# RunhuiWang/DeltaPQ

Measured on AMD Instinct MI355X. Metric: queries/sec, SIFT1M-shaped m=8 k=256 topk=100, higher is better.
Workload: dtype f64 sum of f32 table entries (u8 code decode; the reference's incremental f64 stack); 1 GPU

## Files before the change

deltapq_amd/csrc/dpq_kernels.hip:

```cpp
#include "dpq_kernels.h"
#include "dpq_wave_decoder.h"

#include <atomic>
#include <type_traits>
#include <cfloat>
#include <cmath>

namespace dpq {

static hipError_t ensure_dynamic_lds(const void* fn, size_t bytes, std::atomic<bool>* done);


__device__ __forceinline__ uint32_t and_or(uint32_t a, uint32_t mask, uint32_t c) {
    uint32_t r;
    asm("v_and_or_b32 %0, %1, %2, %3" : "=v"(r) : "v"(a), "s"(mask), "v"(c));
    return r;
}

__device__ __forceinline__ uint64_t make_key(float d, uint32_t id) {
    return ((uint64_t)__float_as_uint(d) << 32) | (uint64_t)id;
}

__device__ __forceinline__ float lut_min_of(const float* __restrict__ lut_min, size_t q, int M, int m) {
    const float4 p = *reinterpret_cast<const float4*>(lut_min + (q * M + m) * kLutMinParts);
// ... 66 lines not shown
    }
}

template <int M>
__global__ __launch_bounds__(64) void decode_segments_kernel(const DeviceImage img,
                                                              const uint32_t* __restrict__ seg_list,
                                                              uint32_t* __restrict__ out_id,
                                                              uint32_t* __restrict__ out_code) {
    constexpr int W = Cfg<M>::W;
    const int lane = threadIdx.x;
    const uint32_t seg = seg_list ? seg_list[blockIdx.x] : blockIdx.x;
    const int cps = img.chunks_per_segment;
    WaveDecoder<M> dec;
    if (!img.raw) dec.begin_segment(img, seg, lane);
    for (int c = 0; c < cps; ++c) {
        const int64_t node = ((int64_t)seg * cps + c) * 64 + lane;
        uint32_t code[W];
        if (img.raw) {
#pragma unroll
            for (int w = 0; w < W; ++w) code[w] = reinterpret_cast<const uint32_t*>(img.raw)[(size_t)node * W + w];
        } else {
            dec.step(img, node, lane, c + 1 < cps, code);
        }
        const size_t o = ((size_t)blockIdx.x * cps + c) * 64 + lane;
        out_id[o] = node < img.n_local ? img.id_base + (uint32_t)node : 0xffffffffu;
#pragma unroll
        for (int w = 0; w < W; ++w) out_code[W * o + w] = code[w];
    }
}

template <int M>
__global__ __launch_bounds__(256) void decode_list_kernel(const DeviceImage img, const uint32_t* __restrict__ seg_list,
                                                           int n_seg, const uint8_t* __restrict__ relabel,
                                                           uint32_t* __restrict__ out_code) {
    constexpr int W = Cfg<M>::W;
    __builtin_amdgcn_s_setprio(DPQ_UNDER_SCAN_PRIO);
    const int lane = threadIdx.x & 63;
    const int64_t j = (int64_t)blockIdx.x * 4 + (threadIdx.x >> 6);
    if (j >= n_seg) return;
    const int64_t seg = seg_list ? (int64_t)seg_list[j] : j;
    const int cps = img.chunks_per_segment;
    WaveDecoder<M> dec;
    dec.begin_segment(img, (uint32_t)seg, lane);
    for (int c = 0; c < cps; ++c) {
        const int64_t node = (seg * cps + c) * 64 + lane;
        const int64_t out = (j * cps + c) * 64 + lane;
        uint32_t code[W];
        dec.step(img, node, lane, c + 1 < cps, code);
        if (relabel) {
#pragma unroll
            for (int w = 0; w < W; ++w) {
                uint32_t r = 0;
#pragma unroll
                for (int b = 0; b < 4; ++b) r |= (uint32_t)relabel[(4 * w + b) * 256 + ((code[w] >> (8 * b)) & 0xffu)] << (8 * b);
                code[w] = r;
            }
        }
        if constexpr (W == 2)
            reinterpret_cast<uint2*>(out_code)[out] = make_uint2(code[0], code[1]);
        else
            reinterpret_cast<uint4*>(out_code)[out] = make_uint4(code[0], code[1], code[2], code[3]);
    }
}

template <int M>
__device__ __forceinline__ float exact_dist(const float* __restrict__ T, const uint32_t* __restrict__ c, bool fp32_accum) {
    if (fp32_accum) {
        float fsum = 0.0f;
#pragma unroll
        for (int m = 0; m < M; ++m) fsum = __fadd_rn(fsum, T[m * 256 + ((c[m >> 2] >> (8 * (m & 3))) & 0xffu)]);
        return fsum;
    }
    double dsum = 0.0;
#pragma unroll
    for (int m = 0; m < M; ++m) {
        const uint32_t byte = (c[m >> 2] >> (8 * (m & 3))) & 0xffu;
        dsum = __dadd_rn(dsum, (double)T[m * 256 + byte]);
    }
    return (float)dsum;
}

struct FilterScale {
    float s32;
    uint32_t bias;
    double B;
};

template <int M>
__device__ __forceinline__ FilterScale filter_scale(uint64_t key, const float* __restrict__ lut_min, size_t q) {
    using C = Cfg<M>;
    FilterScale r{0.0f, 0u, 0.0};
    double B = 0.0;
#pragma unroll
    for (int mm = 0; mm < M; ++mm) B += (double)lut_min_of(lut_min, q, M, mm);
    const double taup = (double)__uint_as_float((uint32_t)(key >> 32)) * (1.0 + 0x1p-20);
    const double R = taup - B;
    r.B = B;
    if (key != ~0ull && R > 0.0 && R < 1e300) {
        const float s = (float)((double)C::QT / R * (1.0 - 0x1p-20));
        if (s <= FLT_MAX) {
            r.s32 = s;
            r.bias = C::R == 1 ? (uint32_t)C::BIAS : 0u;
        }
    }
    return r;
}

template <int M>
__device__ __forceinline__ float filter_offset(const FilterScale& fs, float min_m, int m) {
    const float mn = fs.s32 != 0.0f ? min_m : 0.0f;
    const double od = (double)mn * (double)fs.s32;
    float of = (float)od;
    if ((double)of < od) of = __uint_as_float(__float_as_uint(of) + 1u);
    const double sd = (m == 0 ? (double)fs.bias : 0.0) - 0.5 - (double)of;
    float sf = (float)sd;
    if ((double)sf > sd) sf = __uint_as_float(__float_as_uint(sf) + (sf > 0.0f ? -1 : 1));
    return sf;
}

template <int M>
__device__ __forceinline__ uint32_t filter_field(float tv, float sc, float of, uint32_t bias_m) {
    using C = Cfg<M>;
    const float fv = fminf(__fmaf_rn(tv, sc, of), (float)C::SAT + (float)bias_m);
    return __builtin_amdgcn_cvt_pk_u8_f32(fv, 0u, 0u);
}

template <int M>
__device__ __forceinline__ void write_filter_fields(uint4* qtab, int slot, const float* T, float sc, const float* of_m,
                                                    uint32_t bias, const uint8_t* __restrict__ relabel, int tid, int nthreads) {
    using C = Cfg<M>;
    constexpr int F = C::F, AB = C::AB, R = C::R, QG = C::QG, NG = C::NG, J = C::J;
    const int group = slot / QG, ls = slot % QG;
    const int f = (ls % (J * F)) / J, acc = (ls / (J * F)) * AB + ls % J;
    const int d = acc / R, tb = f * R + acc % R;
    const int g = d >> 2, c = d & 3;
    unsigned char* base = reinterpret_cast<unsigned char*>(qtab + ((size_t)group * NG + g) * M * 256) + c * 4 + tb;
    for (int e = tid; e < M * 256; e += nthreads) {
        const int m = e >> 8;
        const uint32_t v = T ? filter_field<M>(T[e], sc, of_m[m], m == 0 ? bias : 0u) : C::reject_entry(m);
        const int row = relabel ? (m << 8) + relabel[e] : e;
        base[(size_t)row * 16] = (unsigned char)v;
    }
}

template <int M>
__global__ __launch_bounds__(256) void quantise_kernel(const ScanArgs a) {
    using C = Cfg<M>;
    constexpr int QG = C::QG, NG = C::NG;
    constexpr int TE = M * 256;
    constexpr int NS = 16;
    __shared__ float s_scale[NS], s_off[NS];
    __shared__ int32_t s_row[NS];
    __shared__ uint32_t s_bias[NS];
    const int g = blockIdx.x / M, m = blockIdx.x % M, group = blockIdx.y, k = threadIdx.x;
    if (blockIdx.x == 0 && a.tight_hist)
        for (int i = k; i < QG * kTightWords; i += 256) a.tight_hist[(size_t)group * QG * kTightWords + i] = 0;
    if (k < NS) {
        const int ls = C::slot_of_table(g, k >> 2, k & 3);
        const int slot = group * QG + ls;
        int qq = a.slot_query ? a.slot_query[slot] : (slot < a.n_queries ? slot : -1);
        FilterScale fs{0.0f, 0u, 0.0};
        float mn_m = 0.0f;
        if (qq >= 0 && a.debug_pass != 1) {
            uint64_t key = ~0ull;
            if (a.debug_pass != 2) key = a.thr_key[slot];
            fs = filter_scale<M>(key, a.lut_min, (size_t)qq);
            mn_m = lut_min_of(a.lut_min, (size_t)qq, M, m);
        } else {
            qq = -1;
        }
        const float s32 = fs.s32;
        const uint32_t bias = fs.bias;
        const float of = filter_offset<M>(fs, mn_m, m);
        s_scale[k] = s32;
        s_off[k] = of;
        s_bias[k] = m == 0 ? bias : 0u;
        s_row[k] = qq >= 0 ? qq * TE + m * 256 : -1;
    }
    __syncthreads();
    uint32_t out[4] = {0, 0, 0, 0};
#pragma unroll
    for (int c = 0; c < 4; ++c) {
#pragma unroll
        for (int tb = 0; tb < 4; ++tb) {
            const int i = c * 4 + tb;
            const int row = s_row[i];
            const float sc = s_scale[i], of = s_off[i];
            const uint32_t bias = s_bias[i];
            const float tv = row >= 0 ? a.lut32[(size_t)row + k] : 0.0f;
            const float fv = fminf(__fmaf_rn(tv, sc, of), (float)C::SAT + (float)bias);
            out[c] = row < 0 ? out[c] | (C::reject_entry(m) << (8 * tb))
                             : __builtin_amdgcn_cvt_pk_u8_f32(fv, (uint32_t)tb, out[c]);
        }
    }
    a.qtab[((size_t)group * NG * M + blockIdx.x) * 256 + k] = make_uint4(out[0], out[1], out[2], out[3]);
}

#ifndef DPQ_TIGHT_SLEEP
#define DPQ_TIGHT_SLEEP 32
#endif
#ifndef DPQ_GATHER_PIPE
#define DPQ_GATHER_PIPE 0
#endif

constexpr int kFiltered = 0x1000;

template <int M>
struct ScanLds {
    using C = Cfg<M>;
    static constexpr size_t kTables = (size_t)C::NG * M * 256 * 16;
    static constexpr size_t kThr = kTables;
    static constexpr size_t kBase = kThr + (size_t)C::QG * 8;
    static constexpr size_t kCount = kBase + (size_t)C::QG * 4;
    static constexpr size_t kChecks = kCount + (size_t)C::QG * 4;
    static constexpr size_t kScale = kChecks + 16;
    static constexpr size_t kBdn = kScale + (size_t)C::QG * 4;
    static constexpr size_t kExtra = kBdn + (size_t)C::QG * 4;
    static constexpr size_t kHist = kExtra + (size_t)C::NA * 4;
    static constexpr size_t kQCode = kHist + (size_t)C::QG * kTightBuckets * 2;
    static constexpr size_t kQId = kQCode + (size_t)kScanWaves * C::QCAP * M;
    static constexpr size_t kQMask = kQId + (size_t)kScanWaves * C::QCAP * 4;
    static constexpr size_t kBytes = kQMask + (size_t)kScanWaves * C::QCAP * 4 * C::MD;
    static_assert(kBytes <= 160 * 1024, "one workgroup per CU: 160 KB of LDS");
};

enum { kStPrologue = 0, kStSegment, kStDecode, kStGather, kStFold, kStPush, kStRefine, kStTotal, kStSteps, kStRefines,
       kStWaves, kStEntries, kStCount };

template <int MF, bool PLAIN, bool STAMPS, bool TIGHT>
__global__ __launch_bounds__(kScanThreads, (PLAIN && !STAMPS && (MF & ~kFiltered) <= 8) ? 5 : 4) void scan_kernel(const ScanArgs a) {
    constexpr int M = MF & ~kFiltered;
    constexpr bool FILT = (MF & kFiltered) != 0;
    using C = Cfg<M>;
    constexpr int W = C::W, QG = C::QG, NG = C::NG, NA = C::NA, EB = C::AB, F = C::F, MD = C::MD, QCAP = C::QCAP;
    constexpr int TE = M * 256;
    extern __shared__ __attribute__((aligned(16))) unsigned char smem[];
    uint4* lut = reinterpret_cast<uint4*>(smem);
    uint64_t* s_thr = reinterpret_cast<uint64_t*>(smem + ScanLds<M>::kThr);
    int32_t* s_base = reinterpret_cast<int32_t*>(smem + ScanLds<M>::kBase);
    uint32_t* wg_count = reinterpret_cast<uint32_t*>(smem + ScanLds<M>::kCount);
    uint32_t* wg_checks = reinterpret_cast<uint32_t*>(smem + ScanLds<M>::kChecks);
    uint32_t* wg_next = wg_checks + 1;
    float* s_scale = reinterpret_cast<float*>(smem + ScanLds<M>::kScale);
    float* s_bdn = reinterpret_cast<float*>(smem + ScanLds<M>::kBdn);
    uint32_t* s_extra = reinterpret_cast<uint32_t*>(smem + ScanLds<M>::kExtra);
    uint32_t* s_hist = reinterpret_cast<uint32_t*>(smem + ScanLds<M>::kHist);
    uint32_t* rq_code = reinterpret_cast<uint32_t*>(smem + ScanLds<M>::kQCode) + (size_t)(threadIdx.x >> 6) * QCAP * W;
    uint32_t* rq_id = reinterpret_cast<uint32_t*>(smem + ScanLds<M>::kQId) + (size_t)(threadIdx.x >> 6) * QCAP;
    uint32_t* rq_mask = reinterpret_cast<uint32_t*>(smem + ScanLds<M>::kQMask) + (size_t)(threadIdx.x >> 6) * QCAP * MD;

    const int tid = threadIdx.x;
    const int lane = tid & 63;
    uint64_t st[kStCount] = {};
    uint64_t t_mark = 0, t_start = 0;
    auto stamp = [&](int section) {
        if constexpr (STAMPS) {
            const uint64_t now = __builtin_amdgcn_s_memtime();
            st[section] += now - t_mark;
            t_mark = now;
// ... 254 lines not shown
            if (k.c == 0) {
                k.h_doff = a.img.seg_delta_off[k.seg];
#pragma unroll
                for (int w = 0; w < W; ++w) k.h_stk[w] = 0;
                if (lane < C::LEVELS) {
                    const uint32_t* ck = reinterpret_cast<const uint32_t*>(a.img.seg_ckpt) + ((size_t)k.seg * C::LEVELS + lane) * W;
#pragma unroll
                    for (int w = 0; w < W; ++w) k.h_stk[w] = ck[w];
                }
            }
        }
    };
    uint64_t at = 0;
    auto stage2 = [&](Chunk& k) {
        if (k.seg < 0 || PLAIN) return;
        if (k.c == 0) at = k.h_doff;
        k.ld = WaveDecoder<M>::load_delta(a.img, k.in, node_of(k), at);
    };
    auto successor = [&](const Chunk& k) {
        Chunk n;
        n.seg = k.seg;
        n.pos = k.pos;
        n.c = k.c + 1;
        if (k.seg >= 0 && n.c == cps) {
            n.seg = next_entry();
            n.pos = entry_pos;
            n.c = 0;
        }
        return n;
    };
    Chunk A, B, Cn;
    uint32_t fwA = 0, fwB = 0, fwC = 0;
    auto filter_word = [&](const Chunk& k) -> uint32_t { return k.seg < 0 ? 0u : a.filter[(size_t)node_of(k) >> 5]; };
    A.seg = helper ? -1 : next_entry();
    A.pos = entry_pos;
    A.c = 0;
    stage1(A);
    if constexpr (FILT) fwA = filter_word(A);
    B = successor(A);
    stage1(B);
    if constexpr (FILT) fwB = filter_word(B);
    stage2(A);
    stamp(kStSegment);
    while (A.seg >= 0) {
        if constexpr (PLAIN) {
#pragma unroll
            for (int w = 0; w < W; ++w) asm volatile("" ::"v"(A.raw[w]), "v"(B.raw[w]));
        } else {
            asm volatile("" ::"v"(A.ld.level), "v"(A.ld.mk), "v"(A.ld.par), "v"(A.carry_lane), "v"(B.in.nb), "v"(B.in.mk),
                         "v"(B.in.par), "v"(B.carry_lane));
#pragma unroll
            for (int h = 0; h < W / 2; ++h)
                asm volatile("" ::"v"(A.ld.w[h][0]), "v"(A.ld.w[h][1]), "v"(A.ld.w[h][2]), "v"(A.ld.t[h].x), "v"(A.ld.t[h].y));
#pragma unroll
            for (int w = 0; w < W; ++w) asm volatile("" ::"v"(A.h_stk[w]), "v"(B.h_stk[w]));
        }
        if constexpr (FILT) asm volatile("" ::"v"(fwA), "v"(fwB));
        Cn = successor(B);
        stage2(B);
        stage1(Cn);
        if constexpr (FILT) fwC = filter_word(Cn);
        {
            const int64_t node = node_of(A);
            uint32_t code[W];
            if (PLAIN) {
#pragma unroll
                for (int w = 0; w < W; ++w) code[w] = A.raw[w];
            } else {
                if (A.c == 0) {
#pragma unroll
                    for (int w = 0; w < W; ++w) dec.stk[w] = A.h_stk[w];
                }
                dec.finish(A.ld, lane, A.carry_lane, code);
            }
            if constexpr (STAMPS) {
                st[kStSteps] += 1;
                asm volatile("" ::"v"(code[0]), "v"(code[W - 1]));
            }
            stamp(kStDecode);

            uint32_t acc[NA];
            uint32_t fold_h[MD] = {};
            if constexpr (C::R == 1 && DPQ_GATHER_PIPE > 0) {
                static_assert(NG * 8 == 32 && (DPQ_GATHER_PIPE % 2) == 0 && DPQ_GATHER_PIPE >= 2 && DPQ_GATHER_PIPE <= 14, "window of read pairs");
                uint32_t off[8];
#pragma unroll
                for (int m = 0; m < 8; ++m) off[m] = (code[m >> 2] >> (8 * (m & 3))) & 0xffu;
                uint4 gv[32];
#define DPQ_RD(r) gv[r] = lut[(((r) >> 3) * M + ((r) & 7)) * 256 + off[(r) & 7]]
#pragma unroll
                for (int r = 0; r < DPQ_GATHER_PIPE; r += 2) {
                    DPQ_RD(r);
                    DPQ_RD(r + 1);
                    __builtin_amdgcn_sched_barrier(0);
                }
#pragma unroll
                for (int p = 0; p < 16; ++p) {
                    if (2 * p + DPQ_GATHER_PIPE < 32) {
                        DPQ_RD(2 * p + DPQ_GATHER_PIPE);
                        DPQ_RD(2 * p + DPQ_GATHER_PIPE + 1);
                    }
                    __builtin_amdgcn_sched_barrier(0);
                    const int g = p >> 2;
                    const uint4 x = gv[2 * p], y = gv[2 * p + 1];
                    if ((p & 3) == 0) {
                        acc[4 * g + 0] = x.x + y.x;
                        acc[4 * g + 1] = x.y + y.y;
                        acc[4 * g + 2] = x.z + y.z;
                        acc[4 * g + 3] = x.w + y.w;
                    } else {
                        acc[4 * g + 0] += x.x + y.x;
                        acc[4 * g + 1] += x.y + y.y;
                        acc[4 * g + 2] += x.z + y.z;
                        acc[4 * g + 3] += x.w + y.w;
                    }
                    if ((p & 3) == 3) {
#pragma unroll
                        for (int j = 4 * g; j < 4 * g + 4; ++j)
                            fold_h[j / EB] = and_or(acc[j], C::LOW << (EB - 1), fold_h[j / EB] >> 1);
                    }
                    __builtin_amdgcn_sched_barrier(0);
                }
#undef DPQ_RD
            } else
#pragma unroll
            for (int g = 0; g < NG; ++g) {
                if constexpr (C::R == 1) {
                    uint4 v[8];
#pragma unroll
                    for (int m = 0; m < 8; ++m) {
                        const uint32_t byte = (code[m >> 2] >> (8 * (m & 3))) & 0xffu;
                        v[m] = lut[(g * M + m) * 256 + byte];
                    }
                    acc[4 * g + 0] = ((v[0].x + v[1].x + v[2].x) + v[3].x + v[4].x) + (v[5].x + v[6].x + v[7].x);
                    acc[4 * g + 1] = ((v[0].y + v[1].y + v[2].y) + v[3].y + v[4].y) + (v[5].y + v[6].y + v[7].y);
                    acc[4 * g + 2] = ((v[0].z + v[1].z + v[2].z) + v[3].z + v[4].z) + (v[5].z + v[6].z + v[7].z);
                    acc[4 * g + 3] = ((v[0].w + v[1].w + v[2].w) + v[3].w + v[4].w) + (v[5].w + v[6].w + v[7].w);
                } else {
                    uint32_t lo[4], hi[4];
                    if constexpr (TIGHT) {
                        asm volatile("" ::: "memory");
                        const uint4 e0 = reinterpret_cast<const uint4*>(s_extra)[2 * g], e1 = reinterpret_cast<const uint4*>(s_extra)[2 * g + 1];
                        lo[0] = e0.x, hi[0] = e0.y, lo[1] = e0.z, hi[1] = e0.w, lo[2] = e1.x, hi[2] = e1.y, lo[3] = e1.z, hi[3] = e1.w;
                    } else {
#pragma unroll
                        for (int c = 0; c < 4; ++c) lo[c] = hi[c] = (uint32_t)C::BIAS * C::LOW;
                    }
#pragma unroll
                    for (int m0 = 0; m0 < M; m0 += C::PRE) {
                        uint32_t p[4] = {0, 0, 0, 0};
#pragma unroll
                        for (int mm = 0; mm < C::PRE; ++mm) {
                            const int m = m0 + mm;
                            const uint32_t byte = (code[m >> 2] >> (8 * (m & 3))) & 0xffu;
                            const uint4 v = lut[(g * M + m) * 256 + byte];
                            p[0] += v.x, p[1] += v.y, p[2] += v.z, p[3] += v.w;
                        }
#pragma unroll
                        for (int c = 0; c < 4; ++c) {
                            lo[c] += __builtin_amdgcn_perm(0u, p[c], 0x0c020c00u);
                            hi[c] += __builtin_amdgcn_perm(0u, p[c], 0x0c030c01u);
                        }
                    }
#pragma unroll
                    for (int c = 0; c < 4; ++c) {
                        acc[(4 * g + c) * 2 + 0] = lo[c];
                        acc[(4 * g + c) * 2 + 1] = hi[c];
                    }
                }
            }
            if constexpr (STAMPS) {
#pragma unroll
                for (int i = 0; i < NA; ++i) asm volatile("" ::"v"(acc[i]));
            }
            stamp(kStGather);
            bool valid = node < a.img.n_local;
            if constexpr (FILT) valid = valid && ((fwA >> ((uint32_t)node & 31u)) & 1u) != 0u;
            uint64_t pend = 0;
#pragma unroll
            for (int h = 0; h < MD; ++h) {
                uint32_t fail = 0;
                if constexpr (C::R == 1 && DPQ_GATHER_PIPE > 0) {
                    fail = fold_h[h];
                } else {
#pragma unroll
                    for (int j = 0; j < C::J; ++j) fail = and_or(acc[EB * h + j], C::LOW << (EB - 1), fail >> 1);
                }
                fail >>= EB - C::J;
                pend |= (uint64_t)(valid ? (~fail & live) : 0u) << (32 * h);
            }
            const uint64_t pushing = __ballot(pend != 0);
            stamp(kStFold);
            if (pushing) {
                const int cnt = (int)__popcll(pushing);
                while (rq_n + cnt > QCAP) {
                    refine(min(rq_n, 64));
                    stamp(kStRefine);
                }
                if (pend != 0) {
                    int pos = rq_head + rq_n + (int)mbcnt64(pushing, 0);
                    pos = pos >= QCAP ? pos - QCAP : pos;
#pragma unroll
                    for (int w = 0; w < W; ++w) rq_code[pos * W + w] = code[w];
                    rq_id[pos] = a.img.id_base + (uint32_t)node;
                    rq_mask[pos * MD] = (uint32_t)pend;
                    if constexpr (MD == 2) rq_mask[pos * MD + 1] = (uint32_t)(pend >> 32);
                }
                rq_n += cnt;
                stamp(kStPush);
            }
        }
        A = B;
        B = Cn;
        if constexpr (FILT) fwA = fwB, fwB = fwC;
    }
    while (rq_n > 0) refine(min(rq_n, 64));
    stamp(kStRefine);
    if constexpr (TIGHT) {
        if (helper) {
            for (;;) {
// ... 377 lines not shown
#define DPQ_S1_SKIP 0
#endif
#ifndef DPQ_S1_U8
#define DPQ_S1_U8 1
#endif
#ifndef DPQ_S1_PAIR
#define DPQ_S1_PAIR 2
#endif
#ifndef DPQ_S1_DEPTH
#define DPQ_S1_DEPTH 1
#endif
#ifndef DPQ_S1_THREADS
#define DPQ_S1_THREADS 1024
#endif
constexpr int kS1Threads = DPQ_S1_THREADS, kS1Waves = kS1Threads / 64;
constexpr int kS1Buckets = 64;
static_assert((DPQ_S1_QT >> 2) < kS1Buckets && DPQ_S1_QT <= 253, "a lane per bucket; 8 entries of 255 must reject");

struct S1Lds {
    static constexpr size_t kTq = 0;
    static constexpr size_t kSel = kTq + 256 * 32 * 8;
    static constexpr size_t kStack = kSel + 16 * 32 * 4;
    static constexpr size_t kT32 = kStack + (size_t)kS1Waves * 8 * 64 * 8;
    static constexpr size_t kShare = kT32 + 8 * 256 * 4;
    static constexpr size_t kHist = kShare + 48;
    static constexpr size_t kBytes = kHist + 64 * 4;
};
static_assert(S1Lds::kBytes <= 160 * 1024 && S1Lds::kTq == 0, "one workgroup per CU; the bound rows sit at LDS offset 0");

#define DPQ_LDS __attribute__((address_space(3)))
__device__ __forceinline__ uint2 lds_ld64(uint32_t off) {
    const uint64_t v = *(const DPQ_LDS uint64_t*)(uintptr_t)off;
    return make_uint2((uint32_t)v, (uint32_t)(v >> 32));
}
__device__ __forceinline__ uint32_t lds_ld32(uint32_t off) { return *(const DPQ_LDS uint32_t*)(uintptr_t)off; }
__device__ __forceinline__ void lds_st64(uint32_t off, uint2 v) { *(DPQ_LDS uint64_t*)(uintptr_t)off = ((uint64_t)v.y << 32) | v.x; }
__device__ __forceinline__ uint32_t lds_ld8(uint32_t off) { return *(const DPQ_LDS uint8_t*)(uintptr_t)off; }
__device__ __forceinline__ uint2 lds_ld64_whole(uint32_t off) {
    const uint64_t v = *(const volatile DPQ_LDS uint64_t*)(uintptr_t)off;
    return make_uint2((uint32_t)v, (uint32_t)(v >> 32));
}

__device__ __forceinline__ uint32_t s1_nibble_sel(uint32_t nib) {
    uint32_t sel = 0, rank = 0;
#pragma unroll
    for (int i = 0; i < 4; ++i) {
        const bool set = (nib >> i) & 1u;
        sel |= (set ? rank : 4u + i) << (8 * i);
        rank += set ? 1u : 0u;
    }
    return sel;
}

__device__ __forceinline__ uint32_t wave_inclusive_sum(uint32_t v) {
    v += (uint32_t)__builtin_amdgcn_update_dpp(0, (int)v, 0x111, 0xf, 0xf, false);
    v += (uint32_t)__builtin_amdgcn_update_dpp(0, (int)v, 0x112, 0xf, 0xf, false);
    v += (uint32_t)__builtin_amdgcn_update_dpp(0, (int)v, 0x114, 0xf, 0xf, false);
    v += (uint32_t)__builtin_amdgcn_update_dpp(0, (int)v, 0x118, 0xf, 0xf, false);
    v += (uint32_t)__builtin_amdgcn_update_dpp(0, (int)v, 0x142, 0xa, 0xf, false);
    v += (uint32_t)__builtin_amdgcn_update_dpp(0, (int)v, 0x143, 0xc, 0xf, false);
    return v;
}

__global__ __launch_bounds__(kS1Threads) void strand1_kernel(const ScanArgs a) {
    constexpr int M = 8, TE = M * 256, GROUPS = kRunLen / kPhaseLen, D = DPQ_S1_DEPTH, QT = DPQ_S1_QT;
    extern __shared__ __attribute__((aligned(16))) unsigned char smem[];
    const int tid = threadIdx.x, lane = tid & 63, wave = tid >> 6;
    const int slot = blockIdx.y;
    const int qq = a.slot_query ? (slot < a.n_queries ? a.slot_query[slot] : -1) : (slot < a.n_queries ? slot : -1);
    if (qq < 0) return;
    if ((uint32_t)(uintptr_t)(DPQ_LDS unsigned char*)smem != 0u) __builtin_trap();
    uint64_t thr = a.thr_key[slot];
    unsigned long long* const stp = a.stamps ? a.stamps + ((size_t)blockIdx.x * kS1Waves + wave) * 16 : nullptr;
    int n_stamp = 0;
    unsigned long long slow_ticks = 0, slow_entries = 0;
    auto stamp = [&]() {
        if (stp && n_stamp < 14) {
            const unsigned long long t = (__builtin_amdgcn_s_memrealtime() & 0xffffffffffull) | ((__builtin_amdgcn_s_memtime() >> 10) << 40);
            if (lane == 0) stp[n_stamp] = t;
            ++n_stamp;
        }
    };
    stamp();
    FilterScale fs{0.0f, 0u, 0.0};
    float min_m[M];
    {
        double B = 0.0;
#pragma unroll
        for (int m = 0; m < M; ++m) {
            min_m[m] = lut_min_of(a.lut_min, (size_t)qq, M, m);
            B += (double)min_m[m];
        }
        const double taup = (double)__uint_as_float((uint32_t)(thr >> 32)) * (1.0 + 0x1p-20);
        const double R = taup - B;
        fs.B = B;
        if (thr != ~0ull && R > 0.0 && R < 1e300) fs.s32 = (float)((double)QT / R * (1.0 - 0x1p-20));
        if (!(fs.s32 <= FLT_MAX)) fs.s32 = 0.0f;
    }
    const float sc = fs.s32, bdn = __double2float_rd(fs.B);
    const int dbg = a.debug_pass >= 16 ? a.debug_pass - 16 : 0;
    uint32_t* hist = a.tight_hist && sc != 0.0f && !(dbg & 4) ? a.tight_hist + (size_t)slot * (kS1Replicas * kS1ReplicaWords) : nullptr;
    int cut = QT;

    float* T32 = reinterpret_cast<float*>(smem + S1Lds::kT32);
    {
        const float* src = a.lut32 + (size_t)qq * TE;
        for (int i = tid; i < TE; i += kS1Threads) T32[i] = src[i];
        if (tid < 16 * 32) reinterpret_cast<uint32_t*>(smem + S1Lds::kSel)[tid] = s1_nibble_sel((uint32_t)tid >> 5);
        __syncthreads();
        uint2* qtmp = reinterpret_cast<uint2*>(smem + S1Lds::kStack);
        if (tid < 256) {
            uint32_t lo = 0, hi = 0;
#pragma unroll
            for (int m = 0; m < M; ++m) {
                const float of = filter_offset<M>(fs, min_m[m], 1);
                const float fv = sc != 0.0f ? fminf(__fmaf_rn(T32[m * 256 + tid], sc, of), 255.0f) : 0.0f;
                if (m < 4)
                    lo = __builtin_amdgcn_cvt_pk_u8_f32(fv, (uint32_t)m, lo);
                else
                    hi = __builtin_amdgcn_cvt_pk_u8_f32(fv, (uint32_t)(m - 4), hi);
            }
            qtmp[tid] = make_uint2(lo, hi);
        }
        __syncthreads();
        uint2* Tq = reinterpret_cast<uint2*>(smem + S1Lds::kTq);
        if constexpr (DPQ_S1_U8) {
            uint32_t* Tw = reinterpret_cast<uint32_t*>(smem + S1Lds::kTq);
            for (int w = tid; w < 256 * 64; w += kS1Threads) {
                const uint2 row = qtmp[w >> 6];
                Tw[w] = ((w >> 5) & 1) ? row.y : row.x;
            }
        } else {
            for (int w = tid; w < 256 * 32; w += kS1Threads) Tq[w] = qtmp[w >> 5];
        }
        if (tid == 0) {
            *reinterpret_cast<uint32_t*>(smem + S1Lds::kShare) = (uint32_t)QT;
            *reinterpret_cast<unsigned long long*>(smem + S1Lds::kShare + 8) = thr;
            *reinterpret_cast<uint4*>(smem + S1Lds::kShare + 16) = make_uint4(0u, 0u, 0u, 0u);
            *reinterpret_cast<uint4*>(smem + S1Lds::kShare + 32) = make_uint4(0u, 0u, 0u, 0u);
        }
        if (tid < 64) reinterpret_cast<uint32_t*>(smem + S1Lds::kHist)[tid] = 0u;
        __syncthreads();
    }

    stamp();
    const uint32_t lane8 = (uint32_t)(lane & 31) * (DPQ_S1_U8 ? 4u : 8u);
    const uint32_t lane_sel = (uint32_t)S1Lds::kSel + (uint32_t)(lane & 31) * 4u;
    const uint32_t lane_stk = (uint32_t)S1Lds::kStack + (uint32_t)wave * (8 * 64 * 8) + (uint32_t)lane * 8u - 512u;

    DPQ_LDS uint32_t* const sh_cut = (DPQ_LDS uint32_t*)(uintptr_t)S1Lds::kShare;
    DPQ_LDS unsigned long long* const sh_thr = (DPQ_LDS unsigned long long*)(uintptr_t)(S1Lds::kShare + 8);
    DPQ_LDS uint32_t* const sh_count = (DPQ_LDS uint32_t*)(uintptr_t)(S1Lds::kShare + 16);
    DPQ_LDS uint32_t* const sh_done = (DPQ_LDS uint32_t*)(uintptr_t)(S1Lds::kShare + 20);
    DPQ_LDS uint32_t* const sh_next = (DPQ_LDS uint32_t*)(uintptr_t)(S1Lds::kShare + 24);
    DPQ_LDS uint32_t* const sh_stat = (DPQ_LDS uint32_t*)(uintptr_t)(S1Lds::kShare + 32);
    DPQ_LDS uint32_t* const sh_hist = (DPQ_LDS uint32_t*)(uintptr_t)S1Lds::kHist;
    auto look = [&]() {
        const uint32_t mine = __hip_atomic_exchange(sh_hist + lane, 0u, __ATOMIC_RELAXED, __HIP_MEMORY_SCOPE_WORKGROUP);
        if (mine) atomicAdd(hist + (blockIdx.x % kS1Replicas) * kS1ReplicaWords + lane, mine);
        uint32_t v = 0;
#pragma unroll
        for (int r = 0; r < kS1Replicas; ++r) v += __hip_atomic_load(hist + r * kS1ReplicaWords + lane, __ATOMIC_RELAXED, __HIP_MEMORY_SCOPE_AGENT);
        uint32_t incl = v;
#pragma unroll
        for (int o = 1; o < 64; o <<= 1) {
            const uint32_t up = (uint32_t)__shfl_up((int)incl, o);
            if (lane >= o) incl += up;
// ... 740 lines not shown

    if (tid == 0) {
        uint64_t t = n_valid >= a.top_k ? kth : ~0ull;
        if (a.keep_thr) t = min(t, a.thr_key[slot]);
        a.thr_key[slot] = t;
    }

    int p2 = 1;
    while (p2 < kk) p2 <<= 1;
    if (a.final_pass)
        for (int i = tid; i < p2; i += THREADS) wkeys[i] = ~0ull;
    __syncthreads();
    for (int i = tid; i < n; i += THREADS) {
        const uint64_t key = keys[i];
        if (kk > 0 && key <= kth) {
            const uint32_t pos = atomicAdd(&counters[0], 1u);
            if (pos < (uint32_t)KP) wkeys[pos] = key;
        }
    }
    __syncthreads();

    mark(3);
    if (!a.final_pass) {
        for (int i = tid; i < kk; i += THREADS) cand[i] = wkeys[i];
        if (tid == 0) region_n[0] = (uint32_t)kk;
        return;
    }

    if (kk <= DPQ_RANK_BY_COUNT_MAX) {
        for (int i = tid; i < kk; i += THREADS) {
            const uint64_t mine = wkeys[i];
            int rank = 0;
            for (int j = 0; j < kk; ++j) rank += wkeys[j] < mine ? 1 : 0;
            const size_t o = (size_t)q * a.top_k + rank;
            a.out_ids[o] = report_id((uint32_t)(mine & 0xffffffffu), a.n_codes_total);
            a.out_dists[o] = __uint_as_float((uint32_t)(mine >> 32));
        }
        for (int r = kk + tid; r < a.top_k; r += THREADS) {
            const size_t o = (size_t)q * a.top_k + r;
            a.out_ids[o] = -1;
            a.out_dists[o] = INFINITY;
        }
        mark(4);
        if (a.stamps && tid == 0) a.stamps[(size_t)slot * 8 + 7] = __builtin_amdgcn_s_memrealtime();
        return;
    }
    block_bitonic_sort(wkeys, p2, tid, THREADS);
    for (int r = tid; r < a.top_k; r += THREADS) {
        const size_t o = (size_t)q * a.top_k + r;
        if (r < kk) {
            a.out_ids[o] = report_id((uint32_t)(wkeys[r] & 0xffffffffu), a.n_codes_total);
            a.out_dists[o] = __uint_as_float((uint32_t)(wkeys[r] >> 32));
        } else {
            a.out_ids[o] = -1;
            a.out_dists[o] = INFINITY;
        }
    }
}

constexpr int kBootThreads = 512;
constexpr int kBootCells = 736;
constexpr int kBootCellsPerThread = 2;
constexpr int kBootBatch = 6;

template <int MF, int V>
__global__ __launch_bounds__(kBootThreads, (MF & ~kFiltered) <= 8 ? 8 : 6) void bootstrap_kernel(const BootArgs a) {
    constexpr int M = MF & ~kFiltered;
    constexpr bool FILT = (MF & kFiltered) != 0;
    constexpr int W = Cfg<M>::W;
    constexpr int TE = M * 256;
    extern __shared__ __attribute__((aligned(16))) unsigned char smem[];
    uint32_t* keys = reinterpret_cast<uint32_t*>(smem);
    float* T = reinterpret_cast<float*>(smem + (size_t)a.cap * 4);
    uint32_t* cstart = reinterpret_cast<uint32_t*>(T + TE);
    uint16_t* pre = reinterpret_cast<uint16_t*>(cstart + kBootCells);
    uint8_t* ord = reinterpret_cast<uint8_t*>(pre + 1024 + 4);
    uint32_t* hist = reinterpret_cast<uint32_t*>(ord + 2 * kBootPairs * 256);
    uint32_t* bcast = hist + 264;
    uint32_t* wave_sum = bcast + 2;

    const int slot = blockIdx.x, tid = threadIdx.x, lane = tid & 63, wave = tid >> 6;
    const int q = a.slot_query ? a.slot_query[slot] : (slot < a.n_queries ? slot : -1);
    if (q < 0) {
        if (a.qtab) write_filter_fields<M>(a.qtab, slot, nullptr, 0.0f, nullptr, 0u, nullptr, tid, kBootThreads);
        return;
    }
    if (a.stamps && tid == 0) a.stamps[(size_t)slot * 8 + 6] = __builtin_amdgcn_s_memrealtime();
    if (tid == 0) a.cand_count[(size_t)slot * kRegionStride] = 0;
    {
        const float4* src = reinterpret_cast<const float4*>(a.lut32 + (size_t)q * TE);
        for (int i = tid; i < TE / 4; i += kBootThreads) reinterpret_cast<float4*>(T)[i] = src[i];
    }
    __syncthreads();
    auto mark = [&](int i) {
        if (a.stamps && tid == 0) a.stamps[(size_t)slot * 8 + i] = __builtin_amdgcn_s_memtime();
    };
    mark(0);
    if (a.nbr) {
        const int sl = wave;
        const int sub = 2 * (sl >> 1) * (M / 8) + (sl & 1);
        const float* row = T + sub * 256;
        uint32_t best = 0xffffffffu;
#pragma unroll
        for (int j = 0; j < 4; ++j)
            best = min(best, (__float_as_uint(row[lane + 64 * j]) & 0xffffff00u) | (uint32_t)(lane + 64 * j));
#pragma unroll
        for (int off = 32; off > 0; off >>= 1) best = min(best, (uint32_t)__shfl_xor((int)best, off, 64));
        const uint8_t* nb = a.nbr + ((size_t)sl * 256 + (best & 0xffu)) * 256;
        uint32_t cand[4];
#pragma unroll
        for (int j = 0; j < 4; ++j) cand[j] = nb[lane + 64 * j];
        uint32_t key = (__float_as_uint(row[cand[0]]) & 0xffffff00u) | cand[0];
#pragma unroll
        for (int k = 2; k <= 64; k <<= 1) {
#pragma unroll
            for (int j = k >> 1; j > 0; j >>= 1) {
                const uint32_t other = (uint32_t)__shfl_xor((int)key, j, 64);
                const bool take_min = ((lane & k) == 0) == ((lane & j) == 0);
                key = take_min ? min(key, other) : max(key, other);
            }
        }
        ord[sl * 256 + lane] = (uint8_t)(key & 0xffu);
#pragma unroll
        for (int j = 1; j < 4; ++j) ord[sl * 256 + lane + 64 * j] = (uint8_t)cand[j];
    } else {
        const int h = tid >> 8, i = tid & 255;
        uint32_t key[4];
#pragma unroll
        for (int r = 0; r < 4; ++r) {
            const int sl = 4 * h + r, sub = 2 * (sl >> 1) * (M / 8) + (sl & 1);
            key[r] = (__float_as_uint(T[sub * 256 + i]) & 0xffffff00u) | (uint32_t)i;
        }
        uint32_t* xch = keys;
#pragma unroll
        for (int k = 2; k <= 256; k <<= 1) {
#pragma unroll
            for (int j = k >> 1; j > 0; j >>= 1) {
                uint32_t other[4];
                if (j >= 64) {
#pragma unroll
                    for (int r = 0; r < 4; ++r) xch[r * kBootThreads + tid] = key[r];
                    __syncthreads();
#pragma unroll
                    for (int r = 0; r < 4; ++r) other[r] = xch[r * kBootThreads + (tid ^ j)];
                    __syncthreads();
                } else {
#pragma unroll
                    for (int r = 0; r < 4; ++r) other[r] = (uint32_t)__shfl_xor((int)key[r], j, 64);
                }
                const bool take_min = ((i & k) == 0) == ((i & j) == 0);
#pragma unroll
                for (int r = 0; r < 4; ++r) key[r] = take_min ? min(key[r], other[r]) : max(key[r], other[r]);
            }
        }
#pragma unroll
        for (int r = 0; r < 4; ++r) ord[(4 * h + r) * 256 + i] = (uint8_t)(key[r] & 0xffu);
    }
    __syncthreads();
    mark(1);

    int have = 0;
    int evaluated = 0;
    int rounds = 0;
    uint32_t key_lo = 0xffffffffu, key_hi = 0u;
    const int P = a.n_classes;
    const int p_shift = P == 4 ? 2 : 0;
    int w0 = 0;
// ... 72 lines not shown
                for (int r = 0; r < kBootBatch; ++r) fw[r] = a.filter[id[r] >> 5];
#pragma unroll
                for (int r = 0; r < kBootBatch; ++r) {
                    const int v = v0 + tid + r * kBootThreads;
                    float d = 0.0f;
#pragma unroll
                    for (int m = 0; m < M; ++m) d += T[m * 256 + ((code[r][m >> 2] >> (8 * (m & 3))) & 0xffu)];
                    if (v < take && ((fw[r] >> (id[r] & 31u)) & 1u)) {
                        const uint32_t slot_i = atomicAdd(&s_kept, 1u);
                        if (slot_i < (uint32_t)a.cap) {
                            keys[slot_i] = __float_as_uint(d);
                            key_lo = min(key_lo, __float_as_uint(d));
                            key_hi = max(key_hi, __float_as_uint(d));
                        }
                    }
                }
                __syncthreads();
                const uint32_t kept = s_kept;
                __syncthreads();
                if (kept >= (uint32_t)a.cap) {
                    v0 += kBootThreads * kBootBatch;
                    break;
                }
            }
            evaluated += min(v0, take);
            have = (int)min(s_kept, (uint32_t)a.cap);
        } else {
        const int take = min((int)total, a.cap - have);
        for (int v0 = 0; v0 < take; v0 += kBootThreads * kBootBatch) {
            uint32_t e[kBootBatch], code[kBootBatch][W];
#pragma unroll
            for (int r = 0; r < kBootBatch; ++r) {
                const int v = min(v0 + tid + r * kBootThreads, take - 1);
                int pos = 0;
#pragma unroll
                for (int step = 512; step > 0; step >>= 1)
                    pos += (uint32_t)pre[pos + step] <= (uint32_t)v ? step : 0;
                e[r] = cstart[pos] + ((uint32_t)v - pre[pos]);
            }
#pragma unroll
            for (int r = 0; r < kBootBatch; ++r) {
#pragma unroll
                for (int w = 0; w < W; ++w) code[r][w] = a.mi_code[(size_t)e[r] * W + w];
            }
#pragma unroll
            for (int r = 0; r < kBootBatch; ++r) {
                const int v = v0 + tid + r * kBootThreads;
                float d = 0.0f;
#pragma unroll
                for (int m = 0; m < M; ++m) d += T[m * 256 + ((code[r][m >> 2] >> (8 * (m & 3))) & 0xffu)];
                if (v < take) {
                    keys[have + v] = __float_as_uint(d);
                    if constexpr (V & 1) {
                        key_lo = min(key_lo, __float_as_uint(d));
                        key_hi = max(key_hi, __float_as_uint(d));
                    }
                }
            }
        }
        have += take;
        }
        ++rounds;
        w0 += n_w;
        __syncthreads();
        mark(3);
        if (have >= a.cap) break;
    }
    if (a.stamps && tid == 0) a.stamps[(size_t)slot * 8 + 5] = (unsigned long long)rounds;
    uint64_t kth = ~0ull;
    if (have >= a.top_k) {
        uint32_t dbits;
        if constexpr (V & 1)
            dbits = block_kth_bound_u32<10>(keys, have, a.top_k, key_lo, key_hi, cstart, hist, tid, kBootThreads);
        else
            dbits = (uint32_t)block_radix_select(keys, have, a.top_k, hist, bcast, tid, kBootThreads);
        const float bound = __double2float_ru((double)__uint_as_float(dbits) * (1.0 + 0x1p-19));
        kth = ((uint64_t)__float_as_uint(bound) << 32) | 0xffffffffull;
    }
    if (tid == 0) a.thr_key[slot] = kth;
    mark(4);
    if (a.qtab) {
        __shared__ float s_of[M];
        __shared__ float s_scale;
        __shared__ uint32_t s_bias;
        if (tid < M) {
            const FilterScale fs = filter_scale<M>(kth, a.lut_min, (size_t)q);
            s_of[tid] = filter_offset<M>(fs, lut_min_of(a.lut_min, (size_t)q, M, tid), tid);
            if (tid == 0) {
                s_scale = fs.s32;
                s_bias = fs.bias;
            }
        }
        __syncthreads();
        write_filter_fields<M>(a.qtab, slot, T, s_scale, s_of, s_bias, a.relabel, tid, kBootThreads);
    }
    if (a.stamps && tid == 0) a.stamps[(size_t)slot * 8 + 7] = __builtin_amdgcn_s_memrealtime();
}

__global__ __launch_bounds__(256) void filter_ids_kernel(const uint32_t* __restrict__ ids, int n,
                                                         const uint32_t* __restrict__ filter, uint32_t id_base,
                                                         uint32_t* __restrict__ out) {
    const int i = blockIdx.x * 256 + threadIdx.x;
    if (i >= n) return;
    const uint32_t id = ids[i];
    const uint32_t l = id - id_base;
    out[i] = id != 0xffffffffu && ((filter[l >> 5] >> (l & 31u)) & 1u) ? id : 0xffffffffu;
}

hipError_t launch_filter_ids(const uint32_t* ids, int n, const uint32_t* filter, uint32_t id_base, uint32_t* out,
                             hipStream_t stream) {
    if (n <= 0) return hipSuccess;
    if (!ids || !filter || !out) return hipErrorInvalidValue;
    hipLaunchKernelGGL(filter_ids_kernel, dim3((unsigned)((n + 255) / 256)), dim3(256), 0, stream, ids, n, filter, id_base, out);
    return hipGetLastError();
}

size_t bootstrap_lds_bytes(int M, int cap) {
    return (size_t)cap * 4 + (size_t)M * 256 * 4 + (size_t)kBootCells * 4 + (1024 + 4) * 2 + 2 * kBootPairs * 256 + (264 + 2 + 8) * 4;
}

template <int V>
static hipError_t launch_bootstrap_variant(const BootArgs& a, int M, int n_slots, size_t lds, hipStream_t stream) {
    if (M == 8) {
        static std::atomic<bool> done[64] = {};
        hipError_t e = ensure_dynamic_lds(reinterpret_cast<const void*>(&bootstrap_kernel<8, V>), 128 * 1024, done);
        if (e != hipSuccess) return e;
        hipLaunchKernelGGL((bootstrap_kernel<8, V>), dim3((unsigned)n_slots), dim3(kBootThreads), lds, stream, a);
    } else if (M == 16) {
        static std::atomic<bool> done[64] = {};
        hipError_t e = ensure_dynamic_lds(reinterpret_cast<const void*>(&bootstrap_kernel<16, V>), 128 * 1024, done);
        if (e != hipSuccess) return e;
        hipLaunchKernelGGL((bootstrap_kernel<16, V>), dim3((unsigned)n_slots), dim3(kBootThreads), lds, stream, a);
    } else {
        return hipErrorInvalidValue;
    }
    return hipGetLastError();
}

hipError_t launch_bootstrap(const BootArgs& a, int M, int n_slots, hipStream_t stream) {
    if (n_slots <= 0) return hipSuccess;
    if (a.cap < a.top_k || a.cap < 2048 || a.cap > 16384 || !a.cell_start || (a.n_classes != 1 && a.n_classes != kBootPairs))
        return hipErrorInvalidValue;
    const size_t lds = bootstrap_lds_bytes(M, a.cap);
    if (a.filter) {
        if (a.eval_cap < 1) return hipErrorInvalidValue;
        if (M == 8) {
            static std::atomic<bool> done[64] = {};
            hipError_t e = ensure_dynamic_lds(reinterpret_cast<const void*>(&bootstrap_kernel<8 | kFiltered, 1>), 128 * 1024, done);
            if (e != hipSuccess) return e;
            hipLaunchKernelGGL((bootstrap_kernel<8 | kFiltered, 1>), dim3((unsigned)n_slots), dim3(kBootThreads), lds, stream, a);
        } else if (M == 16) {
            static std::atomic<bool> done[64] = {};
            hipError_t e = ensure_dynamic_lds(reinterpret_cast<const void*>(&bootstrap_kernel<16 | kFiltered, 1>), 128 * 1024, done);
            if (e != hipSuccess) return e;
            hipLaunchKernelGGL((bootstrap_kernel<16 | kFiltered, 1>), dim3((unsigned)n_slots), dim3(kBootThreads), lds, stream, a);
        } else {
            return hipErrorInvalidValue;
        }
        return hipGetLastError();
    }
    return (a.variant & 1) ? launch_bootstrap_variant<1>(a, M, n_slots, lds, stream)
                           : launch_bootstrap_variant<0>(a, M, n_slots, lds, stream);
}

__global__ __launch_bounds__(kSelectThreads) void merge_kernel(const int32_t* __restrict__ ids,
                                                                const float* __restrict__ dists, int n_lists, int nq,
                                                                int top_k, int row_stride, int32_t* __restrict__ out_ids,
                                                                float* __restrict__ out_dists) {
    extern __shared__ __attribute__((aligned(16))) unsigned char smem[];
    uint64_t* v = reinterpret_cast<uint64_t*>(smem);
    const int q = blockIdx.x, tid = threadIdx.x;
    const int n = n_lists * top_k;
    for (int i = tid; i < n; i += kSelectThreads) {
        const int l = i / top_k, r = i % top_k;
        const size_t o = ((size_t)l * nq + q) * row_stride + r;
        const int32_t id = ids[o];
        v[i] = id >= 0 ? make_key(dists[o], (uint32_t)id) : ~0ull;
// ... 487 lines not shown
```

deltapq_amd/csrc/dpq_wave_decoder.h:

```cpp
#pragma once
#include "dpq_kernels.h"

namespace dpq {

__device__ __forceinline__ uint32_t bperm(int src_lane, uint32_t v) {
    return (uint32_t)__builtin_amdgcn_ds_bpermute(src_lane << 2, (int)v);
}

__device__ __forceinline__ uint32_t mbcnt64(uint64_t m, uint32_t acc) {
    return __builtin_amdgcn_mbcnt_hi((uint32_t)(m >> 32), __builtin_amdgcn_mbcnt_lo((uint32_t)m, acc));
}


template <int M>
struct Cfg {
    static constexpr int W = M / 4;
    static constexpr int LEVELS = M <= 8 ? 8 : 16;
    static constexpr int JUMPS = M <= 8 ? 3 : 4;
    static constexpr int PLANES = M <= 8 ? 4 : 5;
    static constexpr int EB = 8;
    static constexpr int AB = M <= 8 ? 8 : 16;
    static constexpr int R = AB / EB;
    static constexpr int F = 32 / AB;
    static constexpr int NG = M <= 8 ? 4 : 2;
    static constexpr int NA = NG * 4 * R;
    static constexpr int QG = NA * F;
    static constexpr int J = NA < AB ? NA : AB;
    static constexpr int MD = (NA + AB - 1) / AB;
#ifndef DPQ_QT16
#define DPQ_QT16 250
#define DPQ_SAT16 63
#define DPQ_PRE16 4
#endif
#ifndef DPQ_QT8
#define DPQ_QT8 64
#define DPQ_SAT8 23
#endif
    static constexpr int QT = M <= 8 ? DPQ_QT8 : DPQ_QT16;
    static constexpr int SAT = M <= 8 ? DPQ_SAT8 : DPQ_SAT16;
    static constexpr int XMAX = kTightBuckets - 1;
#ifndef DPQ_XU8
#define DPQ_XU8 1
#endif
#ifndef DPQ_XU16
#define DPQ_XU16 6
#endif
    static constexpr int XU = M <= 8 ? DPQ_XU8 : DPQ_XU16;
    static constexpr int BIAS = (1 << (AB - 1)) - 1 - (QT + 1);
    static constexpr int FIELD_MAX = (1 << EB) - 1;
    static_assert(BIAS >= 0 && M * SAT + BIAS + XMAX * XU < (1 << AB), "a field sum must not carry into its neighbour");
    static_assert(XMAX * XU < QT, "cuts stay above zero");
    static constexpr int PRE = R == 1 ? M : DPQ_PRE16;
    static_assert(R == 1 || (PRE * SAT <= FIELD_MAX && M * SAT > QT + 1 && M % PRE == 0), "byte sums of PRE entries; all-SAT rejects");
    static constexpr uint32_t LOW = AB == 8 ? 0x01010101u : 0x00010001u;
    __host__ __device__ static constexpr int slot_of(int acc, int f) { return (acc / AB) * (J * F) + f * J + acc % AB; }
    __host__ __device__ static constexpr int slot_of_table(int g, int c, int tb) {
        return slot_of((4 * g + c) * R + tb % R, tb / R);
    }
    __host__ __device__ static constexpr uint32_t reject_entry(int m) {
        return R == 1 ? (m == 0 ? (uint32_t)FIELD_MAX : 0u) : (uint32_t)SAT;
    }
    static constexpr int QE_BYTES = 4 * W + 4 + 4 * MD;
    static constexpr int QCAP = M <= 8 ? 88 : 80;
    static_assert(QCAP >= 64 + 16, "a step pushes up to 64 entries");
};

struct DecodeTable {
    uint32_t e[256][2];
    constexpr DecodeTable() : e() {
        for (int b = 0; b < 256; ++b) {
            uint32_t sel[2] = {0, 0};
            uint32_t rank = 0;
            for (int m = 0; m < 8; ++m) {
                const bool set = (b >> m) & 1;
                sel[m >> 2] |= (set ? rank : 0x0cu) << (8 * (m & 3));
                rank += set ? 1u : 0u;
            }
            e[b][0] = sel[0];
            e[b][1] = sel[1];
        }
    }
};
__device__ const DecodeTable g_dtab{};

__device__ __forceinline__ uint32_t own_sel(uint32_t nib) {
    return 0x07060504u - ((nib * 0x00810204u) & 0x04040404u);
}

template <int M>
struct WaveDecoder {
    static constexpr int W = Cfg<M>::W;
    static constexpr int LEVELS = Cfg<M>::LEVELS;
    uint32_t stk[W];
    uint64_t doff;

    __device__ __forceinline__ void begin_segment(const DeviceImage& img, uint32_t seg, int lane) {
        doff = img.seg_delta_off[seg];
#pragma unroll
        for (int w = 0; w < W; ++w) stk[w] = 0;
        if (lane < LEVELS) {
            const uint32_t* ck = reinterpret_cast<const uint32_t*>(img.seg_ckpt) + ((size_t)seg * LEVELS + lane) * W;
#pragma unroll
            for (int w = 0; w < W; ++w) stk[w] = ck[w];
        }
    }

    struct In {
        uint32_t nb, mk, par;
    };
    struct Ld {
        uint32_t level, mk, par;
        uint32_t w[W / 2][3], sh[W / 2];
        uint2 t[W / 2];
    };
    __device__ __forceinline__ static In load_in(const DeviceImage& img, int64_t node) {
        In r;
        r.nb = img.nib[node >> 1];
        r.mk = M <= 8 ? (uint32_t)img.mask[node] : (uint32_t)reinterpret_cast<const uint16_t*>(img.mask)[node];
        r.par = img.par[node];
        return r;
    }
    __device__ __forceinline__ static Ld load_delta(const DeviceImage& img, const In& in, int64_t node, uint64_t& at) {
        Ld r;
        r.level = (node & 1) ? (in.nb >> 4) : (in.nb & 15u);
        r.mk = in.mk;
        r.par = in.par;
        const uint32_t pc = __popc(in.mk);
        uint32_t excl = 0, total = 0;
#pragma unroll
        for (int b = Cfg<M>::PLANES - 1; b >= 0; --b) {
            const uint64_t plane = __ballot((pc >> b) & 1u);
            excl = mbcnt64(plane, excl << 1);
            total = (total << 1) + (uint32_t)__popcll(plane);
        }
#pragma unroll
        for (int h = 0; h < W / 2; ++h) {
            const uint32_t skip = h == 0 ? 0u : (uint32_t)__popc(in.mk & 0xffu);
            const uint8_t* dp = img.delta + at + excl + skip;
            const uintptr_t ua = reinterpret_cast<uintptr_t>(dp);
            const uint32_t* wp = reinterpret_cast<const uint32_t*>(ua & ~(uintptr_t)3);
            r.sh[h] = (uint32_t)(ua & 3);
            r.w[h][0] = wp[0];
            r.w[h][1] = wp[1];
// ... 56 lines not shown
```

Baseline: 6.811 million queries/s.

## Raise m=8 filter quantisation resolution using a byte-lerp averaging tree

For the m=8 packed-byte filter, the quantised LUT entries get finer resolution (QT 64→128, SAT 23→46 by default). The per-field sum becomes a tree: two leaf sums of four entries each, combined with v_lerp_u8 averaging so the sum cannot carry into the neighbouring byte. Biases are spread across leaves so each leaf stays in range, and reject entries move to each leaf's first column. The aim is a tighter filter that sends fewer candidates to exact distance. The cost is extra lerp instructions in the hot accumulate loop and a halving rounding step in the comparison.

```diff
diff --git a/deltapq_amd/csrc/dpq_kernels.hip b/deltapq_amd/csrc/dpq_kernels.hip
--- a/deltapq_amd/csrc/dpq_kernels.hip
+++ b/deltapq_amd/csrc/dpq_kernels.hip
@@ -172,14 +172,14 @@
 
 struct FilterScale {
     float s32;
-    uint32_t bias;
+    bool biased;
     double B;
 };
 
 template <int M>
 __device__ __forceinline__ FilterScale filter_scale(uint64_t key, const float* __restrict__ lut_min, size_t q) {
     using C = Cfg<M>;
-    FilterScale r{0.0f, 0u, 0.0};
+    FilterScale r{0.0f, false, 0.0};
     double B = 0.0;
 #pragma unroll
     for (int mm = 0; mm < M; ++mm) B += (double)lut_min_of(lut_min, q, M, mm);
@@ -190,7 +190,7 @@
         const float s = (float)((double)C::QT / R * (1.0 - 0x1p-20));
         if (s <= FLT_MAX) {
             r.s32 = s;
-            r.bias = C::R == 1 ? (uint32_t)C::BIAS : 0u;
+            r.biased = C::R == 1;
         }
     }
     return r;
@@ -202,7 +202,7 @@
     const double od = (double)mn * (double)fs.s32;
     float of = (float)od;
     if ((double)of < od) of = __uint_as_float(__float_as_uint(of) + 1u);
-    const double sd = (m == 0 ? (double)fs.bias : 0.0) - 0.5 - (double)of;
+    const double sd = (fs.biased ? (double)Cfg<M>::bias_of(m) : 0.0) - 0.5 - (double)of;
     float sf = (float)sd;
     if ((double)sf > sd) sf = __uint_as_float(__float_as_uint(sf) + (sf > 0.0f ? -1 : 1));
     return sf;
@@ -217,7 +217,7 @@
 
 template <int M>
 __device__ __forceinline__ void write_filter_fields(uint4* qtab, int slot, const float* T, float sc, const float* of_m,
-                                                    uint32_t bias, const uint8_t* __restrict__ relabel, int tid, int nthreads) {
+                                                    bool biased, const uint8_t* __restrict__ relabel, int tid, int nthreads) {
     using C = Cfg<M>;
     constexpr int F = C::F, AB = C::AB, R = C::R, QG = C::QG, NG = C::NG, J = C::J;
     const int group = slot / QG, ls = slot % QG;
@@ -227,7 +227,7 @@
     unsigned char* base = reinterpret_cast<unsigned char*>(qtab + ((size_t)group * NG + g) * M * 256) + c * 4 + tb;
     for (int e = tid; e < M * 256; e += nthreads) {
         const int m = e >> 8;
-        const uint32_t v = T ? filter_field<M>(T[e], sc, of_m[m], m == 0 ? bias : 0u) : C::reject_entry(m);
+        const uint32_t v = T ? filter_field<M>(T[e], sc, of_m[m], biased ? (uint32_t)C::bias_of(m) : 0u) : C::reject_entry(m);
         const int row = relabel ? (m << 8) + relabel[e] : e;
         base[(size_t)row * 16] = (unsigned char)v;
     }
@@ -249,7 +249,7 @@
         const int ls = C::slot_of_table(g, k >> 2, k & 3);
         const int slot = group * QG + ls;
         int qq = a.slot_query ? a.slot_query[slot] : (slot < a.n_queries ? slot : -1);
-        FilterScale fs{0.0f, 0u, 0.0};
+        FilterScale fs{0.0f, false, 0.0};
         float mn_m = 0.0f;
         if (qq >= 0 && a.debug_pass != 1) {
             uint64_t key = ~0ull;
@@ -260,11 +260,10 @@
             qq = -1;
         }
         const float s32 = fs.s32;
-        const uint32_t bias = fs.bias;
         const float of = filter_offset<M>(fs, mn_m, m);
         s_scale[k] = s32;
         s_off[k] = of;
-        s_bias[k] = m == 0 ? bias : 0u;
+        s_bias[k] = fs.biased ? (uint32_t)C::bias_of(m) : 0u;
         s_row[k] = qq >= 0 ? qq * TE + m * 256 : -1;
     }
     __syncthreads();
@@ -685,6 +684,7 @@
             uint32_t acc[NA];
             uint32_t fold_h[MD] = {};
             if constexpr (C::R == 1 && DPQ_GATHER_PIPE > 0) {
+                static_assert(C::LD == 0, "the rolling window sums plain byte fields: no lerp tree here");
                 static_assert(NG * 8 == 32 && (DPQ_GATHER_PIPE % 2) == 0 && DPQ_GATHER_PIPE >= 2 && DPQ_GATHER_PIPE <= 14, "window of read pairs");
                 uint32_t off[8];
 #pragma unroll
@@ -735,10 +735,25 @@
                         const uint32_t byte = (code[m >> 2] >> (8 * (m & 3))) & 0xffu;
                         v[m] = lut[(g * M + m) * 256 + byte];
                     }
-                    acc[4 * g + 0] = ((v[0].x + v[1].x + v[2].x) + v[3].x + v[4].x) + (v[5].x + v[6].x + v[7].x);
-                    acc[4 * g + 1] = ((v[0].y + v[1].y + v[2].y) + v[3].y + v[4].y) + (v[5].y + v[6].y + v[7].y);
-                    acc[4 * g + 2] = ((v[0].z + v[1].z + v[2].z) + v[3].z + v[4].z) + (v[5].z + v[6].z + v[7].z);
-                    acc[4 * g + 3] = ((v[0].w + v[1].w + v[2].w) + v[3].w + v[4].w) + (v[5].w + v[6].w + v[7].w);
+                    if constexpr (C::LD == 0) {
+                        acc[4 * g + 0] = ((v[0].x + v[1].x + v[2].x) + v[3].x + v[4].x) + (v[5].x + v[6].x + v[7].x);
+                        acc[4 * g + 1] = ((v[0].y + v[1].y + v[2].y) + v[3].y + v[4].y) + (v[5].y + v[6].y + v[7].y);
+                        acc[4 * g + 2] = ((v[0].z + v[1].z + v[2].z) + v[3].z + v[4].z) + (v[5].z + v[6].z + v[7].z);
+                        acc[4 * g + 3] = ((v[0].w + v[1].w + v[2].w) + v[3].w + v[4].w) + (v[5].w + v[6].w + v[7].w);
+                    } else {
+                        auto avg = [](uint32_t x, uint32_t y) { return (uint32_t)__builtin_amdgcn_lerp(x, y, 0u); };
+                        auto tree = [&](uint32_t e0, uint32_t e1, uint32_t e2, uint32_t e3, uint32_t e4, uint32_t e5, uint32_t e6,
+                                        uint32_t e7) {
+                            if constexpr (C::LD == 1)
+                                return avg((e0 + e1 + e2) + e3, (e4 + e5 + e6) + e7);
+                            else
+                                return avg(avg(e0 + e1, e2 + e3), avg(e4 + e5, e6 + e7));
+                        };
+                        acc[4 * g + 0] = tree(v[0].x, v[1].x, v[2].x, v[3].x, v[4].x, v[5].x, v[6].x, v[7].x);
+                        acc[4 * g + 1] = tree(v[0].y, v[1].y, v[2].y, v[3].y, v[4].y, v[5].y, v[6].y, v[7].y);
+                        acc[4 * g + 2] = tree(v[0].z, v[1].z, v[2].z, v[3].z, v[4].z, v[5].z, v[6].z, v[7].z);
+                        acc[4 * g + 3] = tree(v[0].w, v[1].w, v[2].w, v[3].w, v[4].w, v[5].w, v[6].w, v[7].w);
+                    }
                 } else {
                     uint32_t lo[4], hi[4];
                     if constexpr (TIGHT) {
@@ -1282,7 +1297,7 @@
         }
     };
     stamp();
-    FilterScale fs{0.0f, 0u, 0.0};
+    FilterScale fs{0.0f, false, 0.0};
     float min_m[M];
     {
         double B = 0.0;
@@ -2189,7 +2204,7 @@
     const int slot = blockIdx.x, tid = threadIdx.x, lane = tid & 63, wave = tid >> 6;
     const int q = a.slot_query ? a.slot_query[slot] : (slot < a.n_queries ? slot : -1);
     if (q < 0) {
-        if (a.qtab) write_filter_fields<M>(a.qtab, slot, nullptr, 0.0f, nullptr, 0u, nullptr, tid, kBootThreads);
+        if (a.qtab) write_filter_fields<M>(a.qtab, slot, nullptr, 0.0f, nullptr, false, nullptr, tid, kBootThreads);
         return;
     }
     if (a.stamps && tid == 0) a.stamps[(size_t)slot * 8 + 6] = __builtin_amdgcn_s_memrealtime();
@@ -2428,17 +2443,17 @@
     if (a.qtab) {
         __shared__ float s_of[M];
         __shared__ float s_scale;
-        __shared__ uint32_t s_bias;
+        __shared__ bool s_biased;
         if (tid < M) {
             const FilterScale fs = filter_scale<M>(kth, a.lut_min, (size_t)q);
             s_of[tid] = filter_offset<M>(fs, lut_min_of(a.lut_min, (size_t)q, M, tid), tid);
             if (tid == 0) {
                 s_scale = fs.s32;
-                s_bias = fs.bias;
+                s_biased = fs.biased;
             }
         }
         __syncthreads();
-        write_filter_fields<M>(a.qtab, slot, T, s_scale, s_of, s_bias, a.relabel, tid, kBootThreads);
+        write_filter_fields<M>(a.qtab, slot, T, s_scale, s_of, s_biased, a.relabel, tid, kBootThreads);
     }
     if (a.stamps && tid == 0) a.stamps[(size_t)slot * 8 + 7] = __builtin_amdgcn_s_memrealtime();
 }
diff --git a/deltapq_amd/csrc/dpq_wave_decoder.h b/deltapq_amd/csrc/dpq_wave_decoder.h
--- a/deltapq_amd/csrc/dpq_wave_decoder.h
+++ b/deltapq_amd/csrc/dpq_wave_decoder.h
@@ -32,23 +32,55 @@
 #define DPQ_SAT16 63
 #define DPQ_PRE16 4
 #endif
+#ifndef DPQ_LD8
+#define DPQ_LD8 1
+#endif
 #ifndef DPQ_QT8
+#if DPQ_LD8 == 0
 #define DPQ_QT8 64
 #define DPQ_SAT8 23
+#elif DPQ_LD8 == 1
+#define DPQ_QT8 128
+#define DPQ_SAT8 46
+#else
+#define DPQ_QT8 256
+#define DPQ_SAT8 90
+#endif
 #endif
     static constexpr int QT = M <= 8 ? DPQ_QT8 : DPQ_QT16;
     static constexpr int SAT = M <= 8 ? DPQ_SAT8 : DPQ_SAT16;
+    static constexpr int LD = AB == 8 ? DPQ_LD8 : 0;
+    static constexpr int LEAVES = 1 << LD;
+    static constexpr int LEAF = M / LEAVES;
+    static_assert(LD >= 0 && LD <= 2, "a tree of at most two lerp levels: four pair sums");
     static constexpr int XMAX = kTightBuckets - 1;
 #ifndef DPQ_XU8
-#define DPQ_XU8 1
+#define DPQ_XU8 ((DPQ_QT8 * 11 + 350) / 700)
 #endif
 #ifndef DPQ_XU16
 #define DPQ_XU16 6
 #endif
     static constexpr int XU = M <= 8 ? DPQ_XU8 : DPQ_XU16;
-    static constexpr int BIAS = (1 << (AB - 1)) - 1 - (QT + 1);
+    static constexpr int BIAS = LEAVES * ((1 << (AB - 1)) - 1) + (LEAVES - 1) - (QT + 1);
     static constexpr int FIELD_MAX = (1 << EB) - 1;
-    static_assert(BIAS >= 0 && M * SAT + BIAS + XMAX * XU < (1 << AB), "a field sum must not carry into its neighbour");
+    static constexpr int LEAF_ROOM = FIELD_MAX - LEAF * SAT;
+    static constexpr int BIAS0 = R != 1 ? 0 : (BIAS < LEAF_ROOM - XMAX * XU ? BIAS : LEAF_ROOM - XMAX * XU);
+    __host__ __device__ static constexpr int leaf_bias(int l) {
+        constexpr int others = LEAVES > 1 ? LEAVES - 1 : 1;
+        return l == 0 ? BIAS0 : (BIAS - BIAS0) / others + (l - 1 < (BIAS - BIAS0) % others ? 1 : 0);
+    }
+    __host__ __device__ static constexpr int bias_of(int m) { return R == 1 && m % LEAF == 0 ? leaf_bias(m / LEAF) : 0; }
+    __host__ __device__ static constexpr bool leaves_fit() {
+        int sum = 0;
+        for (int l = 0; l < LEAVES; ++l) {
+            const int b = leaf_bias(l);
+            if (b < 0 || LEAF * SAT + b + (l == 0 ? XMAX * XU : 0) > FIELD_MAX) return false;
+            sum += b;
+        }
+        return sum == BIAS;
+    }
+    static_assert(BIAS >= 0 && (R == 1 ? leaves_fit() : M * SAT + BIAS + XMAX * XU < (1 << AB)),
+                  "a field sum (R = 1: a leaf sum) must not carry into its neighbour");
     static_assert(XMAX * XU < QT, "cuts stay above zero");
     static constexpr int PRE = R == 1 ? M : DPQ_PRE16;
     static_assert(R == 1 || (PRE * SAT <= FIELD_MAX && M * SAT > QT + 1 && M % PRE == 0), "byte sums of PRE entries; all-SAT rejects");
@@ -58,7 +90,7 @@
         return slot_of((4 * g + c) * R + tb % R, tb / R);
     }
     __host__ __device__ static constexpr uint32_t reject_entry(int m) {
-        return R == 1 ? (m == 0 ? (uint32_t)FIELD_MAX : 0u) : (uint32_t)SAT;
+        return R == 1 ? (m % LEAF == 0 ? (uint32_t)FIELD_MAX : 0u) : (uint32_t)SAT;
     }
     static constexpr int QE_BYTES = 4 * W + 4 + 4 * MD;
     static constexpr int QCAP = M <= 8 ? 88 : 80;
```

Result: no change. 6.793 million queries/s (-0.3%).
